# pfe-rs/lk-s-2022-estimacija-pokreta

Hardware: AMD Instinct MI355X
Metric: Mpix/s flow (1024x436, bcd_times=4) (higher is better)
Workload: dtype f64; 1 GPU; single 1024x436 Sintel-shape pair per step per GPU, forward only, bcd_times=4 (BASELINE.json configs[1]); cells 64x27, 150 labels/px; pairs_in_flight_per_gpu=7, mode=batch

## Files before the change

lk-s-2022-estimacija-pokreta_amd/csrc/knn_mfma.hip:

```cpp
#include "dflow_common.h"
#include "knn_pca.h"
#include "row_stage.h"

typedef _Float16 half8 __attribute__((ext_vector_type(8)));
typedef float f32x16 __attribute__((ext_vector_type(16)));

#define KM_ALPHA 64.0f
#define KM_K 48
#define KM_KSTEPS (KM_K / 16)
#define KM_KD 40
#define KM_SLOT_N 40
#define KM_SLOT_QE 41
#define KM_SLOT_EN 42
#define KM_SLOT_H 43
#define KM_SLOT_S 45
#define KM_SLOT_ONE 46
#define KM_XSCALE 64.0
#define KM_SSCALE 4096.0
#define KM_NORM2_MAX 30000.0
#define KM_WAVES 8
#define KM_THREADS (64 * KM_WAVES)
#define KM_QPW 64
#define KM_QPB (KM_WAVES * KM_QPW)
#ifndef KM_CHUNK
#define KM_CHUNK 192
#endif
#define KM_PITCH 112
#define KM_SLOTS (KM_PITCH / 16)
#define KM_STAGE_INS ((KM_CHUNK * KM_SLOTS + 63) / 64)
#define KM_ABUF (KM_STAGE_INS * 1024)
#ifndef KM_NBUF
#define KM_NBUF 3
#endif
#define KM_MAXNW ((KM_STAGE_INS + KM_WAVES - 1) / KM_WAVES)
#define KM_SPC (2 * (KM_CHUNK / 32))
#define KM_EVROWS_MAX 96
#define KM_MAXPTS 65535
#define KM_LIST_WORDS(evrows) (2 * (evrows) * 64)
#define KM_ETA 7.62939453125e-6

struct KmGeom {
    Geom g;
    int LP, qwaves;
    int evrows;
    float tphi;
};

__device__ static inline size_t list_id(const KmGeom &a, int qcell, int qwave, int wslot)
{
    const int win = 2 * a.g.win + 1;
    return ((size_t)qcell * a.qwaves + qwave) * (win * win) + wslot;
}

__host__ __device__ static inline int km_pad(int npts) { return (npts + KM_CHUNK - 1) / KM_CHUNK * KM_CHUNK; }
__host__ __device__ static inline int km_ntiles(int npts) { return km_pad(npts) / 32; }
__host__ __device__ static inline size_t km_cell_base(const Geom &g, int ci, int cj)
{
    const int wl = g.x1(g.ncx - 1) - g.x0(g.ncx - 1), hl = g.y1(g.ncy - 1) - g.y0(g.ncy - 1);
    const size_t rowsum = (size_t)(g.ncx - 1) * km_pad(g.cw * g.ch) + km_pad(wl * g.ch);
    const int hj = cj == g.ncy - 1 ? hl : g.ch;
    return (size_t)cj * rowsum + (size_t)ci * km_pad(g.cw * hj);
}
__host__ __device__ static inline size_t km_total_rows(const Geom &g)
{
    const int wl = g.x1(g.ncx - 1) - g.x0(g.ncx - 1), hl = g.y1(g.ncy - 1) - g.y0(g.ncy - 1);
    return km_cell_base(g, 0, g.ncy - 1) + (size_t)(g.ncx - 1) * km_pad(g.cw * hl) + km_pad(wl * hl);
}

__device__ static inline void km_store_sentinel(_Float16 *row)
{
    half8 *o = reinterpret_cast<half8 *>(row);
    const half8 z = {(_Float16)0.0f, (_Float16)0.0f, (_Float16)0.0f, (_Float16)0.0f, (_Float16)0.0f, (_Float16)0.0f, (_Float16)0.0f, (_Float16)0.0f};
    half8 t8 = z;
    t8[KM_SLOT_H - 40] = (_Float16)60000.0f;
#pragma unroll
    for (int k = 0; k < KM_K / 8; k++) o[k] = k == KM_K / 8 - 1 ? t8 : z;
}

__device__ static inline _Float16 km_f16_up(double v) { return (_Float16)(float)(v * 1.001 + 1e-7); }

#define KM_Q_ZERO 1.0f
#define KM_Q_BAD 2.0f
struct KmCellTop { uint32_t idx[5]; float cost[5]; };

#define KM_RHO 2.65e-5
typedef float km_f2p __attribute__((ext_vector_type(2)));
template <typename T>
__global__ void __launch_bounds__(256) knn_prep_kernel(const T *__restrict__ d1, const T *__restrict__ d2, const float *__restrict__ vt,
                                                       _Float16 *__restrict__ h1, _Float16 *__restrict__ h2,
                                                       float2 *__restrict__ qs, float2 *__restrict__ z0, uint8_t *__restrict__ zflag,
                                                       int *__restrict__ cell_bad, Geom g, int qblocks, int cblocks)
{
    const int which = (int)blockIdx.x >= qblocks ? 1 : 0;
    const T *__restrict__ d = which ? d2 : d1;
    _Float16 *__restrict__ h = which ? h2 : h1;
    const int cell = which ? ((int)blockIdx.x - qblocks) / cblocks : 0;
    int pix;
    size_t orow;
    if (which == 0) {
        pix = blockIdx.x * blockDim.x + threadIdx.x;
        if (pix >= g.H * g.W) return;
        orow = (size_t)pix;
    } else {
        const int ci = cell % g.ncx, cj = cell / g.ncx;
        const int cx0 = g.x0(ci), cy0 = g.y0(cj), ccw = g.x1(ci) - cx0, cnpts = ccw * (g.y1(cj) - cy0);
        const int pos = (((int)blockIdx.x - qblocks) % cblocks) * blockDim.x + threadIdx.x;
        if (pos >= km_pad(cnpts)) return;
        orow = km_cell_base(g, ci, cj) + pos;
        const int idx = (pos & 31) * km_ntiles(cnpts) + (pos >> 5);
        if (idx >= cnpts) {
            km_store_sentinel(h + orow * KM_K);
            z0[orow] = make_float2(INFINITY, 0.0f);
            zflag[orow] = 0;
            return;
        }
        pix = (cy0 + idx / ccw) * g.W + cx0 + idx % ccw;
    }
    float x[DFLOW_DESC];
    desc_load_row(x, d, (size_t)pix);
    if (which == 1) {
        const float4 zero[DFLOW_DESC / 4] = {};
        const PairDist zd = pair_dist(x, zero);
        z0[orow] = make_float2(zd.l2, zd.l1());
    }
    double sxall = 0.0;
    bool bad = false;
#pragma unroll
    for (int k = 0; k < DFLOW_DESC; k++) {
        const float sc = KM_ALPHA * x[k];
        bad |= (__float_as_uint(sc) & 0x7FFFFFFFu) >= 0x7F800000u;
        x[k] = sc;
        sxall = fma((double)sc, (double)sc, sxall);
    }
    bad |= !(sxall < KM_NORM2_MAX);
    const bool zero = sxall == 0.0;
    double ss = 0.0, sx = 0.0, se = 0.0;
    auto component = [&](int j) -> _Float16 {
        const km_f2p *__restrict__ vj = reinterpret_cast<const km_f2p *>(vt + (size_t)j * DFLOW_DESC);
        km_f2p acc = {0.0f, 0.0f};
#pragma unroll
        for (int i = 0; i < DFLOW_DESC / 2; i++) acc = __builtin_elementwise_fma(vj[i], (km_f2p){x[2 * i], x[2 * i + 1]}, acc);
        const float y = acc.x + acc.y;
        const _Float16 hv = (_Float16)y;
        const double f = (double)(float)hv, yd = (double)y, er = f - yd;
        ss = fma(f, f, ss); sx = fma(yd, yd, sx); se = fma(er, er, se);
        return hv;
    };
    half8 *o = reinterpret_cast<half8 *>(h + orow * KM_K);
    static_assert(KM_KD % 8 == 0 && KM_KD + 8 == KM_K, "the last 16-byte piece of a row holds the eight bound slots");
#pragma unroll 1
    for (int jo = 0; jo < KM_KD / 8; jo++) {
        half8 r;
#pragma unroll
        for (int j = 0; j < 8; j++) r[j] = component(8 * jo + j);
        o[jo] = r;
    }
    half8 last;
    const double rx = sqrt(sxall), ry = sqrt(sx);
    const double en = sqrt(se) + KM_RHO * rx;
    const double ypl = fmax(0.0, ry - KM_RHO * rx), ypu = ry + KM_RHO * rx;
    const double nd = sqrt(fmax(0.0, sxall * (1.0 + 1.1 * PCA_DELTA_MAX) - ypl * ypl));
    if (which == 0) {
        last[KM_SLOT_N - 40] = -km_f16_up(nd);
        last[KM_SLOT_QE - 40] = -km_f16_up(sqrt(ss) * (1.0 / KM_XSCALE));
        last[KM_SLOT_EN - 40] = -km_f16_up(en * KM_XSCALE);
        last[KM_SLOT_H - 40] = (_Float16)-1.0f; last[KM_SLOT_H + 1 - 40] = (_Float16)-1.0f;
        last[KM_SLOT_S - 40] = (_Float16)(float)(-1.0 / KM_SSCALE);
        last[KM_SLOT_ONE - 40] = (_Float16)0.0f; last[KM_SLOT_ONE + 1 - 40] = (_Float16)0.0f;
        qs[pix] = make_float2(bad ? KM_Q_BAD : zero ? KM_Q_ZERO : 0.0f, (float)(0.5 * sxall * (1.0 + 1.5 * PCA_DELTA_MAX) * 1.0000002));
    } else {
        const double hh = 0.5 * sxall;
        const _Float16 p1 = (_Float16)(float)hh;
        const _Float16 p2 = (_Float16)(float)(hh - (double)(float)p1);
        const double hres = fabs(hh - (double)(float)p1 - (double)(float)p2);
        const double scs = (KM_ETA * 1.001 * hh + 3e-6 * hh + hres) * 1.0004;
        last[KM_SLOT_N - 40] = km_f16_up(nd);
        last[KM_SLOT_QE - 40] = km_f16_up((en + KM_ETA * sqrt(ss)) * KM_XSCALE);
        last[KM_SLOT_EN - 40] = km_f16_up(ypu * (1.0 / KM_XSCALE));
        last[KM_SLOT_H - 40] = p1; last[KM_SLOT_H + 1 - 40] = p2;
        last[KM_SLOT_S - 40] = km_f16_up(scs * KM_SSCALE);
        last[KM_SLOT_ONE - 40] = (_Float16)1.0f; last[KM_SLOT_ONE + 1 - 40] = (_Float16)1.0f;
        zflag[orow] = zero ? 1 : 0;
        if (bad) cell_bad[cell] = 1;
    }
    o[KM_K / 8 - 1] = last;
}

__global__ void __launch_bounds__(256) knn_cell_post_kernel(_Float16 *__restrict__ h2, const float2 *__restrict__ z0,
                                                            const uint8_t *__restrict__ zflag, KmCellTop *__restrict__ ztop, Geom g)
{
    __shared__ int wsum[4];
    __shared__ unsigned long long wmin[4];
    const int ci = blockIdx.x % g.ncx, cj = blockIdx.x / g.ncx;
    const int cnpts = (g.x1(ci) - g.x0(ci)) * (g.y1(cj) - g.y0(cj));
    const int npad = km_pad(cnpts), ntiles = km_ntiles(cnpts);
    const size_t base = km_cell_base(g, ci, cj);
    const int tid = threadIdx.x, lane = tid & 63, wave = tid >> 6;
    int running = 0;
    for (int c0 = 0; c0 < cnpts; c0 += 256) {
        const int idx = c0 + tid;
        const int pos = (idx % ntiles) * 32 + idx / ntiles;
        const bool z = idx < cnpts && zflag[base + pos] != 0;
        const unsigned long long bal = __ballot(z);
        if (lane == 0) wsum[wave] = __popcll(bal);
        __syncthreads();
        int before = running + __popcll(bal & ((1ull << lane) - 1ull));
        int total = 0;
#pragma unroll
        for (int w = 0; w < 4; w++) { before += w < wave ? wsum[w] : 0; total += wsum[w]; }
        if (z && before >= 5) km_store_sentinel(h2 + (base + pos) * KM_K);
        running += total;
        __syncthreads();
    }
    unsigned long long k5[5];
#pragma unroll
    for (int i = 0; i < 5; i++) k5[i] = ~0ull;
    for (int pos = tid; pos < npad; pos += 256) {
        const int idx = (pos & 31) * ntiles + (pos >> 5);
        const float dd = z0[base + pos].x;
        if (idx < cnpts && dd < INFINITY) {
            unsigned long long x = ((unsigned long long)__float_as_uint(dd) << 32) | (unsigned)idx;
#pragma unroll
            for (int i = 0; i < 5; i++) { const bool lt = x < k5[i]; const unsigned long long lo = lt ? x : k5[i]; x = lt ? k5[i] : x; k5[i] = lo; }
        }
    }
    unsigned long long last = 0ull;
    bool first = true;
    for (int r = 0; r < 5; r++) {
        unsigned long long m = ~0ull;
#pragma unroll
        for (int i = 4; i >= 0; i--) if (first || k5[i] > last) m = k5[i];
        for (int off = 32; off > 0; off >>= 1) { const unsigned long long o = __shfl_xor(m, off); m = o < m ? o : m; }
        if (lane == 0) wmin[wave] = m;
        __syncthreads();
        m = wmin[0];
#pragma unroll
        for (int w = 1; w < 4; w++) m = wmin[w] < m ? wmin[w] : m;
        if (tid == 0) {
            const uint32_t idx = m == ~0ull ? 0u : (uint32_t)(m & 0xFFFFFFFFu);
            ztop[blockIdx.x].idx[r] = idx;
            ztop[blockIdx.x].cost[r] = z0[base + (idx % ntiles) * 32 + idx / ntiles].y;
        }
        last = m; first = false;
        __syncthreads();
    }
}

struct KmScreen {
    const _Float16 *h1, *h2;
    const float2 *qs;
    const int *cell_bad;
    uint32_t *ev;
    uint8_t *ev_cnt;
};

__device__ static inline void top5_insert_desc(float (&a)[5], float m)
{
#pragma unroll
    for (int i = 4; i >= 1; i--) a[i] = __builtin_amdgcn_fmed3f(a[i - 1], a[i], m);
    a[0] = fmaxf(a[0], m);
}

__device__ static inline float max16(const f32x16 &v)
{
    float m0 = fmaxf(fmaxf(v[0], v[1]), v[2]), m1 = fmaxf(fmaxf(v[3], v[4]), v[5]);
    float m2 = fmaxf(fmaxf(v[6], v[7]), v[8]), m3 = fmaxf(fmaxf(v[9], v[10]), v[11]);
    float m4 = fmaxf(fmaxf(v[12], v[13]), v[14]);
    return fmaxf(fmaxf(fmaxf(m0, m1), fmaxf(m2, m3)), fmaxf(m4, v[15]));
}

__global__ void __launch_bounds__(KM_THREADS, 4) knn_screen_kernel(KmGeom a, KmScreen p)
{
    extern __shared__ __attribute__((aligned(16))) char smem[];
    char *abuf = smem;

    const Geom g = a.g;
    const int tid = threadIdx.x, lane = tid & 63, wave = tid >> 6;
    const int col = lane & 31, half = lane >> 5;
    const int win = 2 * g.win + 1;
    const int wgs_per_cell = (win * win * a.qwaves + KM_WAVES - 1) / KM_WAVES;
    const int ccell = blockIdx.x / wgs_per_cell, w8 = blockIdx.x % wgs_per_cell;
    const int ci = ccell % g.ncx, cj = ccell / g.ncx;
    int flat = w8 * KM_WAVES + __builtin_amdgcn_readfirstlane(wave);
    int total = 0, qci = -1, qcj = -1, qwave = 0, fqci = -1, fqcj = -1;
    for (int qslot = 0; qslot < win * win; qslot++) {
        const int sci = ci - g.win + qslot / win, scj = cj - g.win + qslot % win;
        if (sci < 0 || sci >= g.ncx || scj < 0 || scj >= g.ncy) continue;
        const int nw = ((g.x1(sci) - g.x0(sci)) * (g.y1(scj) - g.y0(scj)) + KM_QPW - 1) / KM_QPW;
        if (fqci < 0) { fqci = sci; fqcj = scj; }
        if (qci < 0 && flat >= total && flat < total + nw) { qci = sci; qcj = scj; qwave = flat - total; }
        total += nw;
    }
    if (w8 * KM_WAVES >= total) return;
    const bool wave_active = qci >= 0;
    if (!wave_active) { qci = fqci; qcj = fqcj; qwave = 0; }
    const int qcell = qcj * g.ncx + qci;
    const int qx0 = g.x0(qci), qy0 = g.y0(qcj), qcw = g.x1(qci) - qx0, qnpts = qcw * (g.y1(qcj) - qy0);
    const int wslot = g.window(qci, qcj).slot(ci, cj);
    const int cx0 = g.x0(ci), cy0 = g.y0(cj), ccw = g.x1(ci) - cx0, cnpts = ccw * (g.y1(cj) - cy0);
    (void)cx0; (void)cy0;

    half8 bfrag[2][KM_KSTEPS];
    float hq[2];
    bool qzero[2], qbad = false;
#pragma unroll
    for (int gq = 0; gq < 2; gq++) {
        int qi = qwave * KM_QPW + gq * 32 + col;
        if (qi >= qnpts) qi = qnpts - 1;
        const int qpix = (qy0 + qi / qcw) * g.W + qx0 + qi % qcw;
        const half8 *src = reinterpret_cast<const half8 *>(p.h1 + (size_t)qpix * KM_K);
#pragma unroll
        for (int s = 0; s < KM_KSTEPS; s++) bfrag[gq][s] = src[2 * s + half];
        const float2 qq = p.qs[qpix];
        hq[gq] = qq.y;
        qzero[gq] = qq.x == KM_Q_ZERO;
        qbad |= qq.x == KM_Q_BAD;
    }
    const bool list_bad = __ballot(qbad) != 0ull || p.cell_bad[ccell] != 0;

    const int nchunks = (cnpts + KM_CHUNK - 1) / KM_CHUNK;
    const size_t cbase = km_cell_base(g, ci, cj);
    const int wave_u = __builtin_amdgcn_readfirstlane(wave);
    uint32_t soff[KM_MAXNW];
#pragma unroll
    for (int i = 0; i < KM_MAXNW; i++) {
        const int slot = (wave_u + i * KM_WAVES) * 64 + lane;
        int part = slot % KM_SLOTS;
        if (part >= KM_K / 8) part = 0;
        soff[i] = (uint32_t)((slot / KM_SLOTS) * (KM_K * 2) + part * 16);
    }
    const rs_gptr h2cell = (rs_gptr)(p.h2 + cbase * KM_K);
    const int n_w = (KM_STAGE_INS - wave_u + KM_WAVES - 1) / KM_WAVES;
    auto stage = [&](int chunk, int buf) {
        char *base = abuf + (size_t)buf * KM_ABUF + wave_u * 1024;
        const rs_gptr src = h2cell + (size_t)min(chunk, nchunks - 1) * (KM_CHUNK * KM_K * 2);
#pragma unroll
        for (int i = 0; i < KM_MAXNW; i++)
            if (i < KM_MAXNW - 1 || n_w == KM_MAXNW)
                __builtin_amdgcn_global_load_lds((const __attribute__((address_space(1))) void *)(src + soff[i]),
                                                 (__attribute__((address_space(3))) void *)(base + i * KM_WAVES * 1024), 16, 0, 0);
    };

    float a5[2][5];
    int cnt[2] = {0, 0};
    const int evrows = a.evrows;
    const uint32_t evoff[2] = {(uint32_t)lane * 4u, (uint32_t)lane * 4u + (uint32_t)evrows * 256u};
    const size_t lid = list_id(a, qcell, qwave, wslot);
    const __amdgpu_buffer_rsrc_t evrsrc = __builtin_amdgcn_make_buffer_rsrc((void *)(p.ev + lid * KM_LIST_WORDS(a.evrows)), 0, KM_LIST_WORDS(a.evrows) * 4, 0x00020000);

#pragma unroll
    for (int gq = 0; gq < 2; gq++)
#pragma unroll
        for (int i = 0; i < 5; i++) a5[gq][i] = -INFINITY;

    auto wait_ring = [&](int pass) {
        if (pass == 0) {
            if (n_w == KM_MAXNW) asm volatile("s_waitcnt vmcnt(%0)" ::"n"((KM_NBUF - 2) * KM_MAXNW) : "memory");
            else asm volatile("s_waitcnt vmcnt(%0)" ::"n"((KM_NBUF - 2) * (KM_MAXNW - 1)) : "memory");
        } else {
            if (n_w == KM_MAXNW) asm volatile("s_waitcnt vmcnt(%0)" ::"n"((KM_NBUF - 2) * KM_MAXNW + 2 * KM_SPC) : "memory");
            else asm volatile("s_waitcnt vmcnt(%0)" ::"n"((KM_NBUF - 2) * (KM_MAXNW - 1) + 2 * KM_SPC) : "memory");
        }
        __builtin_amdgcn_s_barrier();
    };
    auto dummy_stores = [&]() {
#pragma unroll
        for (int i = 0; i < KM_SPC; i++) __builtin_amdgcn_raw_buffer_store_b32(0u, evrsrc, (int)0xFFFFFF00u, 0, 0);
    };
    auto epi1 = [&](const f32x16 &acc, int gq) { top5_insert_desc(a5[gq], max16(acc)); };
    auto epi2 = [&](const f32x16 &acc, int gq, int tileidx) {
        uint32_t neg = 0u;
#pragma unroll
        for (int r = 15; r >= 0; r--) neg = __builtin_amdgcn_alignbit(neg, __float_as_uint(acc[r]), 31);
        const bool has = neg != 0xFFFFu;
        const uint32_t off = has ? evoff[gq] + ((uint32_t)min(cnt[gq], evrows - 1) << 8) : 0xFFFFFF00u;
        __builtin_amdgcn_raw_buffer_store_b32(neg ^ (((uint32_t)tileidx << 16) | 0xFFFFu), evrsrc, (int)off, 0, 0);
        cnt[gq] += has ? 1 : 0;
    };
    const f32x16 minus_inf = {-INFINITY, -INFINITY, -INFINITY, -INFINITY, -INFINITY, -INFINITY, -INFINITY, -INFINITY,
                              -INFINITY, -INFINITY, -INFINITY, -INFINITY, -INFINITY, -INFINITY, -INFINITY, -INFINITY};
    f32x16 pend;
    int pend_tile = 0;
    auto one_tile = [&](auto passc, const int tileidx, const half8 (&af)[KM_KSTEPS], half8 (&afn)[KM_KSTEPS], const char *arow_next) __attribute__((always_inline)) {
        constexpr int PASS = decltype(passc)::value;
        if (arow_next) {
#pragma unroll
            for (int s = 0; s < KM_KSTEPS; s++) afn[s] = *reinterpret_cast<const half8 *>(arow_next + s * 32);
        }
        __builtin_amdgcn_sched_barrier(0);
        f32x16 acc0 = {0.f, 0.f, 0.f, 0.f, 0.f, 0.f, 0.f, 0.f, 0.f, 0.f, 0.f, 0.f, 0.f, 0.f, 0.f, 0.f};
#pragma unroll
        for (int s = 0; s < KM_KSTEPS; s++) acc0 = __builtin_amdgcn_mfma_f32_32x32x16_f16(af[s], bfrag[0][s], acc0, 0, 0, 0);
        if (PASS == 0) epi1(pend, 1); else epi2(pend, 1, pend_tile);
#pragma unroll
        for (int s = 0; s < KM_KSTEPS; s++) {
            __builtin_amdgcn_sched_group_barrier(0x008, 1, 0);
            __builtin_amdgcn_sched_group_barrier(0x002, PASS == 0 ? 5 : 8, 0);
        }
        __builtin_amdgcn_sched_barrier(0);
        f32x16 acc1 = {0.f, 0.f, 0.f, 0.f, 0.f, 0.f, 0.f, 0.f, 0.f, 0.f, 0.f, 0.f, 0.f, 0.f, 0.f, 0.f};
#pragma unroll
        for (int s = 0; s < KM_KSTEPS; s++) acc1 = __builtin_amdgcn_mfma_f32_32x32x16_f16(af[s], bfrag[1][s], acc1, 0, 0, 0);
        if (PASS == 0) epi1(acc0, 0); else epi2(acc0, 0, tileidx);
#pragma unroll
        for (int s = 0; s < KM_KSTEPS; s++) {
            __builtin_amdgcn_sched_group_barrier(0x008, 1, 1);
            __builtin_amdgcn_sched_group_barrier(0x002, PASS == 0 ? 5 : 8, 1);
        }
        __builtin_amdgcn_sched_barrier(0);
        pend = acc1; pend_tile = tileidx;
    };
    auto tiles = [&](auto passc, const int chunk, const char *ab) __attribute__((always_inline)) {
        static_assert((KM_CHUNK / 32) % 2 == 1 || KM_CHUNK / 32 >= 2, "tiles per chunk");
        half8 afa[KM_KSTEPS], afb[KM_KSTEPS];
        const char *arow = ab + col * KM_PITCH + half * 16;
#pragma unroll
        for (int s = 0; s < KM_KSTEPS; s++) afa[s] = *reinterpret_cast<const half8 *>(arow + s * 32);
        const int tile0 = chunk * (KM_CHUNK / 32);
#pragma unroll 1
        for (int tile = 0; tile + 1 < KM_CHUNK / 32; tile += 2) {
            one_tile(passc, tile0 + tile, afa, afb, arow + (tile + 1) * 32 * KM_PITCH);
            one_tile(passc, tile0 + tile + 1, afb, afa, tile + 2 < KM_CHUNK / 32 ? arow + (tile + 2) * 32 * KM_PITCH : nullptr);
        }
        if ((KM_CHUNK / 32) % 2 == 1) one_tile(passc, tile0 + KM_CHUNK / 32 - 1, afa, afb, nullptr);
    };
    for (int pass = 0; pass < 2; pass++) {
#pragma unroll
        for (int c = 0; c < KM_NBUF - 1; c++) stage(c, c);
        if (n_w == KM_MAXNW) asm volatile("s_waitcnt vmcnt(%0)" ::"n"((KM_NBUF - 2) * KM_MAXNW) : "memory");
        else asm volatile("s_waitcnt vmcnt(%0)" ::"n"((KM_NBUF - 2) * (KM_MAXNW - 1)) : "memory");
        __builtin_amdgcn_s_barrier();
        pend = minus_inf;
        pend_tile = 0;
        if (pass == 1) dummy_stores();
        for (int chunk = 0; chunk < nchunks; chunk++) {
            const int buf = chunk % KM_NBUF;
            stage(chunk + KM_NBUF - 1, (chunk + KM_NBUF - 1) % KM_NBUF);
            const char *ab = abuf + (size_t)buf * KM_ABUF;
            if (wave_active) { if (pass == 0) tiles(IntC<0>(), chunk, ab); else tiles(IntC<1>(), chunk, ab); }
            else if (pass == 1) dummy_stores();
            wait_ring(pass);
        }
        if (wave_active) { if (pass == 0) epi1(pend, 1); else epi2(pend, 1, pend_tile); }
        asm volatile("s_waitcnt vmcnt(0)" ::: "memory");
        __builtin_amdgcn_s_barrier();
        if (pass == 0) {
#pragma unroll
            for (int gq = 0; gq < 2; gq++) {
                float o[5];
#pragma unroll
                for (int i = 0; i < 5; i++) o[i] = __shfl_xor(a5[gq][i], 32);
#pragma unroll
                for (int i = 0; i < 5; i++) top5_insert_desc(a5[gq], o[i]);
                const float a5v = a5[gq][4];
                const float x = a5v - 2.7e-5f * fmaxf(hq[gq] - a5v, 0.0f);
                float th = fmaxf(x - 1e-6f * (fabsf(a5v) + 2.7e-5f * hq[gq]), -55000.0f);
                if (qzero[gq]) th = 60000.0f;
                const float thp = th - 1e-5f * fabsf(th) - 6e-8f;
                if (half == 1) {
                    half8 b2 = bfrag[gq][KM_KSTEPS - 1];
                    b2[KM_SLOT_N - 40] = -b2[KM_SLOT_N - 40];
                    b2[KM_SLOT_QE - 40] = -b2[KM_SLOT_QE - 40];
                    b2[KM_SLOT_EN - 40] = -b2[KM_SLOT_EN - 40];
                    b2[KM_SLOT_S - 40] = -b2[KM_SLOT_S - 40];
                    const _Float16 p1 = (_Float16)thp;
                    const _Float16 p2 = (_Float16)(thp - (float)p1);
                    b2[KM_SLOT_ONE - 40] = -p1; b2[KM_SLOT_ONE + 1 - 40] = -p2;
                    bfrag[gq][KM_KSTEPS - 1] = b2;
                }
            }
        }
    }
    if (!wave_active) return;
#pragma unroll
    for (int gq = 0; gq < 2; gq++) p.ev_cnt[lid * 128 + gq * 64 + lane] = (uint8_t)(list_bad || cnt[gq] >= evrows ? 255 : cnt[gq]);
}

typedef unsigned int km_u4 __attribute__((ext_vector_type(4)));
struct RowDirectH {
    km_u4 r[9];
    __device__ __forceinline__ void init(char *, uint32_t *, int) {}
    __device__ __forceinline__ void issue(rs_gptr base, uint32_t off16, bool act)
    {
        if (act) {
            const __attribute__((address_space(1))) km_u4 *s = reinterpret_cast<const __attribute__((address_space(1))) km_u4 *>(base + ((unsigned long long)off16 << 4));
#pragma unroll
            for (int j = 0; j < 9; j++) r[j] = s[j];
        }
    }
    __device__ __forceinline__ void fetch(float4 (&cv)[17])
    {
        float f[72];
#pragma unroll
        for (int j = 0; j < 9; j++) {
            const dflow_h8 v = __builtin_bit_cast(dflow_h8, r[j]);
#pragma unroll
            for (int i = 0; i < 8; i++) f[8 * j + i] = (float)v[i];
        }
#pragma unroll
        for (int k = 0; k < 17; k++) cv[k] = make_float4(f[4 * k], f[4 * k + 1], f[4 * k + 2], f[4 * k + 3]);
    }
};
template <bool F16> struct RowsOf { typedef RowStage type; static constexpr uint32_t PIECES = 17u; };
template <> struct RowsOf<true> { typedef RowDirectH type; static constexpr uint32_t PIECES = 9u; };

struct KmResolve {
    const void *d1, *d2;
    const uint32_t *ev;
    const uint8_t *ev_cnt;
    const float2 *qs;
    const KmCellTop *ztop;
    uint32_t *proposals;
    float *lcosts;
    int *ovf_count;
    int4 *ovf_list;
    int ovf_cap;
    int *heavy_count;
    int4 *heavy_list;
    int heavy_cap;
};

__device__ static inline void key_insert(unsigned long long (&k)[5], float (&c)[5], unsigned long long x, float xc)
{
#pragma unroll
    for (int i = 0; i < 5; i++) {
        const bool lt = x < k[i];
        const unsigned long long lo = lt ? x : k[i], hi = lt ? k[i] : x;
        const float clo = lt ? xc : c[i], chi = lt ? c[i] : xc;
        k[i] = lo; c[i] = clo; x = hi; xc = chi;
    }
}
static constexpr unsigned long long KM_NO_KEY = 0x7F800000FFFFFFFFull;

__device__ static inline int km_event_cand(int h, int r, int tile, int ntiles) { return (4 * h + (r & 3) + 8 * (r >> 2)) * ntiles + tile; }

template <bool F16>
__device__ __forceinline__ void km_load_query(typename RowsOf<F16>::type &rows, const void *d1, size_t qpix, float (&q)[DFLOW_DESC])
{
    rows.issue((rs_gptr)d1, (uint32_t)qpix * RowsOf<F16>::PIECES, true);
    float4 qv[DFLOW_DESC / 4];
    rows.fetch(qv);
#pragma unroll
    for (int k = 0; k < DFLOW_DESC / 4; k++) { q[4 * k] = qv[k].x; q[4 * k + 1] = qv[k].y; q[4 * k + 2] = qv[k].z; q[4 * k + 3] = qv[k].w; }
}

template <class Rows, class Next>
__device__ __forceinline__ void km_eval(Rows &rows, Next &&next, const float (&q)[DFLOW_DESC], bool act, int idx,
                                        unsigned long long (&keys)[5], float (&costs)[5])
{
    float4 cv[DFLOW_DESC / 4];
    rows.fetch(cv);
    next();
    const float worst = __uint_as_float((unsigned)(keys[4] >> 32));
    const PairDist d = pair_dist(q, cv);
    if (act && !(d.l2 > worst)) key_insert(keys, costs, ((unsigned long long)__float_as_uint(d.l2) << 32) | (unsigned)idx, d.l1());
}

__device__ static inline void km_emit(const KmGeom &a, const KmResolve &p, size_t qpix, int qy, int qx, int cx0, int cy0, int ccw,
                                      int wslot, int j, unsigned long long key, float cost)
{
    const int idx = (int)(key & 0xFFFFFFFFu);
    const int ty = cy0 + idx / ccw, tx = cx0 + idx % ccw;
    p.proposals[qpix * a.LP + 5 * wslot + j] = pack_flow(ty - qy, tx - qx);
    p.lcosts[qpix * a.LP + 5 * wslot + j] = cost < a.tphi ? cost : a.tphi;
}

#ifndef KM_HEAVY_ENTRIES
#define KM_HEAVY_ENTRIES 32
#endif
#define KM_EVLIST2 30
typedef float km_f2 __attribute__((ext_vector_type(2)));
template <bool F16>
__global__ void __launch_bounds__(64, 2) knn_resolve_kernel(KmGeom a, KmResolve p)
{
    const Geom g = a.g;
    const int lane = threadIdx.x, gq = lane >> 5, col = lane & 31;
    const int win = 2 * g.win + 1;
    int b = blockIdx.x;
    const int qwave = b % a.qwaves; b /= a.qwaves;
    const int cir = b % win; const int qcell = b / win;
    const int qci = qcell % g.ncx, qcj = qcell / g.ncx;
    const int ci = qci - g.win + cir;
    if (ci < 0 || ci >= g.ncx) return;
    const int qx0 = g.x0(qci), qy0 = g.y0(qcj), qcw = g.x1(qci) - qx0, qnpts = qcw * (g.y1(qcj) - qy0);
    if (qwave * KM_QPW >= qnpts) return;
    const Geom::Window w = g.window(qci, qcj);
    const int cx0 = g.x0(ci), ccw = g.x1(ci) - cx0;

    __shared__ __attribute__((aligned(1024))) char stage[F16 ? 16 : ROW_STAGE_BYTES];
    __shared__ uint16_t evl[KM_EVLIST2][64];
    __shared__ __attribute__((aligned(16))) uint32_t s_cand[64];
    typename RowsOf<F16>::type rows;
    constexpr uint32_t PIECES = RowsOf<F16>::PIECES;
    rows.init(stage, s_cand, lane);
    float q[DFLOW_DESC];
    int qi = qwave * KM_QPW + lane;
    const bool qvalid = qi < qnpts;
    if (!qvalid) qi = qnpts - 1;
    const int qy = qy0 + qi / qcw, qx = qx0 + qi % qcw;
    const size_t qpix = (size_t)qy * g.W + qx;
    const bool qzero = p.qs[qpix].x == KM_Q_ZERO;
    km_load_query<F16>(rows, p.d1, qpix, q);
    const rs_gptr d2g = (rs_gptr)p.d2;

    int nA_n, nB_n; uint32_t entA_n[4], entB_n[4];
    auto prefetch = [&](int cj) {
        const size_t lid = list_id(a, qcell, qwave, w.slot(ci, cj));
        nA_n = p.ev_cnt[lid * 128 + gq * 64 + col]; nB_n = p.ev_cnt[lid * 128 + gq * 64 + col + 32];
        const uint32_t *ev = p.ev + lid * KM_LIST_WORDS(a.evrows) + (size_t)gq * a.evrows * 64 + col;
#pragma unroll
        for (int e = 0; e < 4; e++) { entA_n[e] = ev[e * 64]; entB_n[e] = ev[e * 64 + 32]; }
    };
    prefetch(w.jmin);
    for (int cj = w.jmin; cj <= w.jmax; cj++) {
        const int wslot = w.slot(ci, cj);
        const size_t lid = list_id(a, qcell, qwave, wslot);
        const int cy0 = g.y0(cj);
        const int ntiles = km_ntiles(ccw * (g.y1(cj) - cy0));
        int nA = nA_n, nB = nB_n;
        bool ovf = nA == 255 || nB == 255;
        const uint32_t *evA = p.ev + (size_t)lid * KM_LIST_WORDS(a.evrows) + (size_t)gq * a.evrows * 64 + col;
        uint32_t entA[4], entB[4];
#pragma unroll
        for (int e = 0; e < 4; e++) { entA[e] = e < nA && !ovf ? entA_n[e] : 0u; entB[e] = e < nB && !ovf ? entB_n[e] : 0u; }
        if (cj < w.jmax) prefetch(cj + 1);
        if (__ballot(ovf)) {
            if (lane == 0) {
                int pos = atomicAdd(p.ovf_count, 1);
                if (pos < p.ovf_cap) p.ovf_list[pos] = make_int4(qcell, qwave * KM_QPW, ci, cj);
            }
            continue;
        }
        bool heavy = false;
        if (nA + nB > KM_HEAVY_ENTRIES) {
            heavy = true;
            if (qvalid) {
                const int pos = atomicAdd(p.heavy_count, 1);
                if (pos < p.heavy_cap) p.heavy_list[pos] = make_int4(qcell, qi, ci, cj); else heavy = false;
            }
            if (heavy) {
                nA = 0; nB = 0;
#pragma unroll
                for (int e = 0; e < 4; e++) { entA[e] = 0u; entB[e] = 0u; }
            }
        }
        unsigned long long keys[5];
        float costs[5];
#pragma unroll
        for (int i = 0; i < 5; i++) { keys[i] = KM_NO_KEY; costs[i] = 0.0f; }
        int done = 0, total;
        do {
        int nev = 0, seen = 0;
        auto expand = [&](uint32_t entry, int h) {
            const int tile = (int)(entry >> 16);
            uint32_t mask = entry & 0xFFFFu;
            while (mask) {
                const int r = __ffs(mask) - 1;
                mask &= mask - 1;
                if (seen >= done && nev < KM_EVLIST2) { evl[nev][lane] = (uint16_t)km_event_cand(h, r, tile, ntiles); nev++; }
                seen++;
            }
        };
#pragma unroll
        for (int e = 0; e < 4; e++) expand(entA[e], 0);
        for (int e = 4; e < nA; e++) expand(evA[e * 64], 0);
#pragma unroll
        for (int e = 0; e < 4; e++) expand(entB[e], 1);
        for (int e = 4; e < nB; e++) expand(evA[e * 64 + 32], 1);
        total = seen;
        auto issue_cand = [&](int e) -> int {
            const bool act = e < nev;
            const int idx = act ? evl[e][lane] : 0;
            rows.issue(d2g, (uint32_t)((cy0 + idx / ccw) * g.W + cx0 + idx % ccw) * PIECES, act);
            return idx;
        };
        if (__ballot(nev > 0)) {
            int e = 0;
            int idx_next = issue_cand(0);
            while (true) {
                const bool act = e < nev;
                const int idx = idx_next;
                e++;
                const bool more = __ballot(e < nev) != 0;
                km_eval(rows, [&] { if (more) idx_next = issue_cand(e); }, q, act, idx, keys, costs);
                if (!more) break;
            }
        }
        done += nev;
        } while (__ballot(done < total));
        if (qzero) {
            const KmCellTop zt = p.ztop[cj * g.ncx + ci];
#pragma unroll
            for (int i = 0; i < 5; i++) { keys[i] = zt.idx[i]; costs[i] = zt.cost[i]; }
        }
        if (qvalid && !heavy) {
#pragma unroll
            for (int j = 0; j < 5; j++) km_emit(a, p, qpix, qy, qx, cx0, cy0, ccw, wslot, j, keys[j], costs[j]);
        }
    }
}

#define KM_HEAVY_CAND 1024
template <bool F16>
__global__ void __launch_bounds__(64, 2) knn_resolve_heavy_kernel(KmGeom a, KmResolve p)
{
    const Geom g = a.g;
    const int lane = threadIdx.x;
    __shared__ __attribute__((aligned(1024))) char stage[F16 ? 16 : ROW_STAGE_BYTES];
    __shared__ __attribute__((aligned(16))) uint32_t s_cand[64];
    __shared__ uint16_t cand[KM_HEAVY_CAND];
    typename RowsOf<F16>::type rows;
    constexpr uint32_t PIECES = RowsOf<F16>::PIECES;
    rows.init(stage, s_cand, lane);
    const int nitems = min(*p.heavy_count, p.heavy_cap);
    const rs_gptr d2g = (rs_gptr)p.d2;
    for (int item = blockIdx.x; item < nitems; item += gridDim.x) {
        const int4 it = p.heavy_list[item];
        const int qcell = it.x, qi = it.y, ci = it.z, cj = it.w;
        const int qci = qcell % g.ncx, qcj = qcell / g.ncx;
        const int qx0 = g.x0(qci), qy0 = g.y0(qcj), qcw = g.x1(qci) - qx0;
        const int qy = qy0 + qi / qcw, qx = qx0 + qi % qcw;
        const size_t qpix = (size_t)qy * g.W + qx;
        const int wslot = g.window(qci, qcj).slot(ci, cj);
        const int cx0 = g.x0(ci), cy0 = g.y0(cj), ccw = g.x1(ci) - cx0;
        const int ntiles = km_ntiles(ccw * (g.y1(cj) - cy0));
        const size_t lid = list_id(a, qcell, qi / KM_QPW, wslot);
        const int ql = qi % KM_QPW, gq = ql >> 5, col = ql & 31;
        const uint32_t *ev = p.ev + (size_t)lid * KM_LIST_WORDS(a.evrows) + (size_t)gq * a.evrows * 64 + col;
        const int nA = p.ev_cnt[lid * 128 + gq * 64 + col], nB = p.ev_cnt[lid * 128 + gq * 64 + col + 32];
        const int te = min(lane, a.evrows - 1);
        const uint32_t pre_a = ev[(size_t)te * 64], pre_b = ev[(size_t)te * 64 + 32];
        float q[DFLOW_DESC];
        km_load_query<F16>(rows, p.d1, qpix, q);
        unsigned long long keys[5];
        float costs[5];
#pragma unroll
        for (int i = 0; i < 5; i++) { keys[i] = KM_NO_KEY; costs[i] = 0.0f; }
        for (int e0 = 0; e0 < nA + nB; e0 += 64) {
            const int t = e0 + lane;
            uint32_t en = 0u; int h = 0;
            const uint32_t shb = (uint32_t)__shfl((int)pre_b, (t - nA) & 63);
            if (t < nA) en = t < 64 ? pre_a : ev[(size_t)t * 64];
            else if (t < nA + nB) { en = t - nA < 64 ? shb : ev[(size_t)(t - nA) * 64 + 32]; h = 1; }
            const int cntl = t < nA + nB ? __popc(en & 0xFFFFu) : 0;
            int incl = cntl;
#pragma unroll
            for (int off = 1; off < 64; off <<= 1) { const int v = __shfl_up(incl, off); if (lane >= off) incl += v; }
            const int nc = __shfl(incl, 63);
            {
                int o = incl - cntl;
                const int tile = (int)(en >> 16);
                uint32_t m = t < nA + nB ? (en & 0xFFFFu) : 0u;
                while (m) { const int r = __ffs(m) - 1; m &= m - 1; cand[o++] = (uint16_t)km_event_cand(h, r, tile, ntiles); }
            }
            asm volatile("s_waitcnt lgkmcnt(0)" ::: "memory");
            auto issue_cand = [&](int c0) -> int {
                const bool act = c0 + lane < nc;
                const int idx = act ? cand[c0 + lane] : 0;
                rows.issue(d2g, (uint32_t)((cy0 + idx / ccw) * g.W + cx0 + idx % ccw) * PIECES, act);
                return idx;
            };
            int idx_next = issue_cand(0);
            for (int c0 = 0; c0 < nc; c0 += 64) {
                const int idx = idx_next;
                km_eval(rows, [&] { if (c0 + 64 < nc) idx_next = issue_cand(c0 + 64); }, q, c0 + lane < nc, idx, keys, costs);
            }
        }
        unsigned long long rkey = KM_NO_KEY;
        float rcost = 0.0f;
        for (int r = 0; r < 5; r++) {
            unsigned long long m = keys[0];
#pragma unroll
            for (int off = 32; off > 0; off >>= 1) { const unsigned long long o = __shfl_xor(m, off); m = o < m ? o : m; }
            const unsigned long long own = __ballot(keys[0] == m && m != KM_NO_KEY);
            float c = 0.0f;
            if (own) {
                const int wl = __ffsll((long long)own) - 1;
                c = __shfl(costs[0], wl);
                if (lane == wl) {
#pragma unroll
                    for (int i = 0; i < 4; i++) { keys[i] = keys[i + 1]; costs[i] = costs[i + 1]; }
                    keys[4] = KM_NO_KEY; costs[4] = 0.0f;
                }
            }
            if (lane == r) { rkey = m; rcost = c; }
        }
        if (lane < 5) km_emit(a, p, qpix, qy, qx, cx0, cy0, ccw, wslot, lane, rkey, rcost);
    }
}

template <int CTRL> __device__ static inline void dpp_lexmin(float &mind, int &best)
{
    const float om = __builtin_bit_cast(float, __builtin_amdgcn_update_dpp(__builtin_bit_cast(int, mind), __builtin_bit_cast(int, mind), CTRL, 0xF, 0xF, false));
    const int ob = __builtin_amdgcn_update_dpp(best, best, CTRL, 0xF, 0xF, false);
    if (om < mind || (om == mind && ob < best)) { mind = om; best = ob; }
}
__global__ void __launch_bounds__(256) knn_finalize_kernel(Geom g, int LP, uint32_t *__restrict__ proposals, float *__restrict__ lcosts,
                                                           int32_t *__restrict__ nprop, int32_t *__restrict__ bestlabels)
{
    const int sub = threadIdx.x & 15;
    const int pix = (blockIdx.x * blockDim.x + threadIdx.x) >> 4;
    const bool ok = pix < g.H * g.W;
    const int px = ok ? pix : 0;
    const int cy = g.celly(px / g.W), cx = g.cellx(px % g.W);
    const int wy = min(g.ncy - 1, cy + g.win) - max(0, cy - g.win) + 1;
    const int wx = min(g.ncx - 1, cx + g.win) - max(0, cx - g.win) + 1;
    const int n = 5 * wy * wx;
    const float *lc = lcosts + (size_t)px * LP;
    float mind = 1000.0f; int best = 0x7fffffff;
    float cs[DFLOW_MAX_LABELS / 16];
#pragma unroll
    for (int j = 0; j < DFLOW_MAX_LABELS / 16; j++) cs[j] = sub + 16 * j < n ? lc[sub + 16 * j] : 1000.0f;
#pragma unroll
    for (int j = 0; j < DFLOW_MAX_LABELS / 16; j++) if (cs[j] < mind) { mind = cs[j]; best = sub + 16 * j; }
    dpp_lexmin<0x101>(mind, best); dpp_lexmin<0x102>(mind, best); dpp_lexmin<0x104>(mind, best); dpp_lexmin<0x108>(mind, best);
    if (ok) {
        if (sub == 0) { nprop[pix] = n; bestlabels[pix] = best == 0x7fffffff ? 0 : best; }
        for (int l = n + sub; l < LP; l += 16) { proposals[(size_t)pix * LP + l] = DFLOW_FILL_PROPOSAL; lcosts[(size_t)pix * LP + l] = DFLOW_FILL_COST; }
    }
}

static size_t num_lists(const dflow_params *p)
{
    Geom g = make_geom(p);
    size_t qwaves = (max_cell_points(g) + KM_QPW - 1) / KM_QPW, win = 2 * g.win + 1;
    return (size_t)g.ncx * g.ncy * qwaves * win * win;
}

#define KM_HEAVY_BLOCKS 2048
#define KM_HEAVY_CAP (1 << 20)
static int km_evrows(const dflow_params *p)
{
    const int tiles = km_ntiles(max_cell_points(make_geom(p)));
    return tiles + 1 < KM_EVROWS_MAX ? tiles + 1 : KM_EVROWS_MAX;
}

struct KmWs {
    _Float16 *h1, *h2;
    float2 *qs, *z0;
    uint8_t *zflag;
    int *ctr;
    int *cell_bad;
    size_t zero_bytes;
    float *vt;
    void *pca_ws;
    KmCellTop *ztop;
    int4 *ovf;
    int4 *heavy;
    uint32_t *ev;
    uint8_t *ev_cnt;
    size_t nl, bytes;
    int evrows;
};

static KmWs km_ws(const dflow_params *p, void *ws)
{
    const Geom g = make_geom(p);
    const size_t N = (size_t)g.H * g.W, rows2 = km_total_rows(g), ncells = (size_t)g.ncx * g.ncy;
    WsCarver c(ws);
    KmWs k;
    k.nl = num_lists(p);
    k.evrows = km_evrows(p);
    k.h1 = c.take<_Float16>(N * KM_K);
    k.h2 = c.take<_Float16>(rows2 * KM_K);
    k.qs = c.take<float2>(N);
    k.z0 = c.take<float2>(rows2);
    k.zflag = c.take<uint8_t>(rows2);
    k.zero_bytes = 256 + ncells * sizeof(int);
    k.ctr = c.take<int>(k.zero_bytes / sizeof(int));
    k.cell_bad = k.ctr + 256 / sizeof(int);
    k.vt = c.take<float>(DFLOW_DESC * DFLOW_DESC);
    k.pca_ws = c.take<char>(knn_pca_ws_bytes());
    k.ztop = c.take<KmCellTop>(ncells);
    k.ovf = c.take<int4>(k.nl);
    k.heavy = c.take<int4>(KM_HEAVY_CAP);
    k.ev = c.take<uint32_t>(k.nl * KM_LIST_WORDS(k.evrows));
    k.ev_cnt = c.take<uint8_t>(k.nl * 128);
    k.bytes = c.bytes;
    return k;
}

size_t knn_mfma_ws_bytes(const dflow_params *p) { return km_ws(p, nullptr).bytes; }

static KmGeom km_geom(const dflow_params *p, const KmWs &k)
{
    KmGeom a;
    a.g = make_geom(p); a.LP = p->label_pitch; a.tphi = p->tphi;
    a.qwaves = (max_cell_points(a.g) + KM_QPW - 1) / KM_QPW;
    a.evrows = k.evrows;
    return a;
}

bool knn_mfma_supported(const dflow_params *p)
{
    Geom g = make_geom(p);
    return max_cell_points(g) <= KM_MAXPTS && p->window >= 0 && p->window <= 2;
}

#define KM_MARK(i) do { if (tev) DFLOW_HIP(hipEventRecord(tev[i], s)); } while (0)
int launch_knn_mfma(const dflow_params *p, const void *d1, const void *d2, uint32_t *proposals, float *lcosts,
                    int32_t *nprop, int32_t *bestlabels, void *ws, hipStream_t s, hipEvent_t *tev)
{
    Geom g = make_geom(p);
    const size_t N = (size_t)g.H * g.W;
    const KmWs k = km_ws(p, ws);
    DFLOW_HIP(hipMemsetAsync(k.ctr, 0, k.zero_bytes, s));
    int nb = (int)((N + 255) / 256);
    KM_MARK(0);
    int rc = launch_knn_pca(p, d2, k.vt, k.ctr + 1, k.pca_ws, s);
    if (rc) return rc;
    KM_MARK(1);
    const int cblocks = (km_pad(max_cell_points(g)) + 255) / 256;
    with_descr_type(p, [&](auto d) {
        using T = typename decltype(d)::T;
        hipLaunchKernelGGL(knn_prep_kernel<T>, dim3(nb + cblocks * g.ncx * g.ncy), dim3(256), 0, s, (const T *)d1, (const T *)d2, (const float *)k.vt,
                           k.h1, k.h2, k.qs, k.z0, k.zflag, k.cell_bad, g, nb, cblocks);
    });
    hipLaunchKernelGGL(knn_cell_post_kernel, dim3(g.ncx * g.ncy), dim3(256), 0, s, k.h2, (const float2 *)k.z0, (const uint8_t *)k.zflag, k.ztop, g);
    rc = dflow_check_launch("knn_cell_post_kernel");
    if (rc) return rc;

    KM_MARK(2);
    const KmGeom a = km_geom(p, k);
    int win = 2 * g.win + 1;
    int wgs_per_cell = (win * win * a.qwaves + KM_WAVES - 1) / KM_WAVES;
    KmScreen sc;
    sc.h1 = k.h1; sc.h2 = k.h2; sc.qs = k.qs; sc.cell_bad = k.cell_bad; sc.ev = k.ev; sc.ev_cnt = k.ev_cnt;
    size_t shmem = (size_t)KM_NBUF * KM_ABUF;
    hipLaunchKernelGGL(knn_screen_kernel, dim3(g.ncx * g.ncy * wgs_per_cell), dim3(KM_THREADS), shmem, s, a, sc);
    rc = dflow_check_launch("knn_screen_kernel");
    if (rc) return rc;
    KM_MARK(3);
    KmResolve rs;
    rs.d1 = d1; rs.d2 = d2; rs.ev = k.ev; rs.ev_cnt = k.ev_cnt; rs.qs = k.qs; rs.ztop = k.ztop; rs.proposals = proposals; rs.lcosts = lcosts;
    rs.ovf_count = k.ctr; rs.ovf_list = k.ovf; rs.ovf_cap = (int)k.nl;
    rs.heavy_count = k.ctr + 2; rs.heavy_list = k.heavy; rs.heavy_cap = KM_HEAVY_CAP;
    const dim3 rgrid((unsigned)(g.ncx * g.ncy * win * a.qwaves));
    with_descr_type(p, [&](auto d) { hipLaunchKernelGGL(knn_resolve_kernel<decltype(d)::F16>, rgrid, dim3(64), 0, s, a, rs); });
    rc = dflow_check_launch("knn_resolve_kernel");
    if (rc) return rc;
    with_descr_type(p, [&](auto d) { hipLaunchKernelGGL(knn_resolve_heavy_kernel<decltype(d)::F16>, dim3(KM_HEAVY_BLOCKS), dim3(64), 0, s, a, rs); });
    rc = dflow_check_launch("knn_resolve_heavy_kernel");
    if (rc) return rc;
    KM_MARK(4);
    rc = launch_knn_fix(p, d1, d2, proposals, lcosts, k.ctr, k.ovf, (int)k.nl, k.ctr + 1, s);
    if (rc) return rc;
    KM_MARK(5);
    hipLaunchKernelGGL(knn_finalize_kernel, dim3((unsigned)((N * 16 + 255) / 256)), dim3(256), 0, s, g, a.LP, proposals, lcosts, nprop, bestlabels);
    KM_MARK(6);
    return dflow_check_launch("knn_finalize_kernel");
}
#undef KM_MARK

__global__ void __launch_bounds__(128) knn_stats_lists_kernel(KmGeom a, const uint32_t *__restrict__ ev, const uint8_t *__restrict__ ev_cnt,
                                                              unsigned long long *__restrict__ out)
{
    const Geom g = a.g;
    const int evrows = a.evrows, win = 2 * g.win + 1;
    const size_t lid = blockIdx.x;
    {
        const int wslot = (int)(lid % (size_t)(win * win)), qwave = (int)(lid / (win * win) % a.qwaves), qcell = (int)(lid / (win * win) / a.qwaves);
        const int qci = qcell % g.ncx, qcj = qcell / g.ncx;
        const Geom::Window w = g.window(qci, qcj);
        const int qnpts = (g.x1(qci) - g.x0(qci)) * (g.y1(qcj) - g.y0(qcj));
        if (qwave * KM_QPW >= qnpts || wslot >= (w.imax - w.imin + 1) * (w.jmax - w.jmin + 1)) return;
    }
    const int gq = threadIdx.x >> 6, lane = threadIdx.x & 63;
    const int cnt = ev_cnt[lid * 128 + threadIdx.x];
    unsigned long long entries = 0, events = 0;
    if (cnt != 255) {
        entries = (unsigned long long)cnt;
        const uint32_t *e = ev + lid * KM_LIST_WORDS(evrows) + (size_t)gq * evrows * 64 + lane;
        for (int i = 0; i < cnt; i++) events += (unsigned long long)__popc(e[i * 64] & 0xFFFFu);
    }
    unsigned long long mx = entries;
    for (int off = 32; off > 0; off >>= 1) { entries += __shfl_xor(entries, off); events += __shfl_xor(events, off); const unsigned long long o = __shfl_xor(mx, off); mx = o > mx ? o : mx; }
    if (lane == 0) { atomicAdd(out + 0, entries); atomicAdd(out + 1, events); atomicMax(out + 2, mx); }
}

__global__ void __launch_bounds__(256) knn_stats_rows_kernel(const float2 *__restrict__ qs, int npix, const uint8_t *__restrict__ zflag,
                                                             const _Float16 *__restrict__ h2, size_t rows2, unsigned long long *__restrict__ out)
{
    const size_t i = (size_t)blockIdx.x * blockDim.x + threadIdx.x;
    const bool zq = i < (size_t)npix && qs[i].x == KM_Q_ZERO, bq = i < (size_t)npix && qs[i].x == KM_Q_BAD;
    const bool zc = i < rows2 && zflag[i] != 0;
    const bool removed = zc && h2[i * KM_K + KM_SLOT_H] == (_Float16)60000.0f;
    const unsigned long long b0 = __ballot(zq), b1 = __ballot(bq), b2 = __ballot(zc), b3 = __ballot(removed);
    if ((threadIdx.x & 63) == 0) {
        if (b0) atomicAdd(out + 3, (unsigned long long)__popcll(b0));
        if (b1) atomicAdd(out + 4, (unsigned long long)__popcll(b1));
        if (b2) atomicAdd(out + 5, (unsigned long long)__popcll(b2));
        if (b3) atomicAdd(out + 6, (unsigned long long)__popcll(b3));
    }
}

int knn_mfma_stats(const dflow_params *p, void *ws, hipStream_t s, int64_t *h_out)
{
    const KmWs k = km_ws(p, ws);
    const Geom g = make_geom(p);
    const size_t N = (size_t)g.H * g.W, rows2 = km_total_rows(g);
    unsigned long long *dev = (unsigned long long *)(k.ctr + 16);
    DFLOW_HIP(hipMemsetAsync(dev, 0, 8 * sizeof(unsigned long long), s));
    const KmGeom a = km_geom(p, k);
    hipLaunchKernelGGL(knn_stats_lists_kernel, dim3((unsigned)k.nl), dim3(128), 0, s, a, (const uint32_t *)k.ev, (const uint8_t *)k.ev_cnt, dev);
    const size_t m = N > rows2 ? N : rows2;
    hipLaunchKernelGGL(knn_stats_rows_kernel, dim3((unsigned)((m + 255) / 256)), dim3(256), 0, s, (const float2 *)k.qs, (int)N, (const uint8_t *)k.zflag,
                       (const _Float16 *)k.h2, rows2, dev);
    int rc = dflow_check_launch("knn_stats kernels");
    if (rc) return rc;
    unsigned long long c[8];
    int ctr[4];
    DFLOW_HIP(hipMemcpyAsync(c, dev, sizeof(c), hipMemcpyDeviceToHost, s));
    DFLOW_HIP(hipMemcpyAsync(ctr, k.ctr, sizeof(ctr), hipMemcpyDeviceToHost, s));
    DFLOW_HIP(hipStreamSynchronize(s));
    long long pairs = 0;
    for (int qcj = 0; qcj < g.ncy; qcj++)
        for (int qci = 0; qci < g.ncx; qci++) {
            const long long qn = (long long)(g.x1(qci) - g.x0(qci)) * (g.y1(qcj) - g.y0(qcj));
            const Geom::Window w = g.window(qci, qcj);
            pairs += qn * (w.imax - w.imin + 1) * (w.jmax - w.jmin + 1);
        }
    h_out[0] = ctr[0]; h_out[1] = ctr[1]; h_out[2] = (int64_t)k.nl; h_out[3] = (int64_t)c[0]; h_out[4] = (int64_t)c[1]; h_out[5] = (int64_t)c[2];
    h_out[6] = (int64_t)c[3]; h_out[7] = (int64_t)c[4]; h_out[8] = (int64_t)c[5]; h_out[9] = (int64_t)c[6]; h_out[10] = pairs; h_out[11] = k.evrows;
    h_out[12] = ctr[2] < KM_HEAVY_CAP ? ctr[2] : KM_HEAVY_CAP;
    h_out[13] = ctr[2] > KM_HEAVY_CAP ? ctr[2] - KM_HEAVY_CAP : 0;
    return DFLOW_OK;
}

double knn_mfma_issued(const dflow_params *p)
{
    Geom g = make_geom(p);
    double n = 0.0;
    for (int qcj = 0; qcj < g.ncy; qcj++)
        for (int qci = 0; qci < g.ncx; qci++) {
            const int qnpts = (g.x1(qci) - g.x0(qci)) * (g.y1(qcj) - g.y0(qcj));
            const int qgroups = 2 * ((qnpts + KM_QPW - 1) / KM_QPW);
            for (int ci = qci - g.win; ci <= qci + g.win; ci++)
                for (int cj = qcj - g.win; cj <= qcj + g.win; cj++) {
                    if (ci < 0 || ci >= g.ncx || cj < 0 || cj >= g.ncy) continue;
                    const int cnpts = (g.x1(ci) - g.x0(ci)) * (g.y1(cj) - g.y0(cj));
                    n += (double)qgroups * km_ntiles(cnpts) * 2.0 * KM_KSTEPS;
                }
        }
    return n;
}
```

Before: 40.90 Mpix/s.

## Restructure kNN MFMA chunk ring to stage one chunk ahead with optional wave lag

Reworks the LDS staging ring in the MFMA kNN kernel. It now prefetches only the next chunk instead of NBUF-1 ahead, waits on vmcnt(0) or just the pending store count, and walks tiles by a global tile index that wraps around the contiguous ring. It adds an optional lag for the upper half of the waves so that their reads skew against the lower half, and it sizes the dummy stores to match the real epilogue stores so the vmcnt bookkeeping stays consistent. The aim is simpler, tighter synchronization and staggered wave progress. The risk is less prefetch depth and more exposed global latency.

```diff
diff --git a/lk-s-2022-estimacija-pokreta_amd/csrc/knn_mfma.hip b/lk-s-2022-estimacija-pokreta_amd/csrc/knn_mfma.hip
--- a/lk-s-2022-estimacija-pokreta_amd/csrc/knn_mfma.hip
+++ b/lk-s-2022-estimacija-pokreta_amd/csrc/knn_mfma.hip
@@ -32,8 +32,19 @@
 #ifndef KM_NBUF
 #define KM_NBUF 3
 #endif
+#ifndef KM_LAG
+#define KM_LAG 0
+#endif
+#define KM_TPC (KM_CHUNK / 32)
+#define KM_TILE_BYTES (32 * KM_PITCH)
+#define KM_RING_TILES (KM_NBUF * KM_TPC)
 #define KM_MAXNW ((KM_STAGE_INS + KM_WAVES - 1) / KM_WAVES)
-#define KM_SPC (2 * (KM_CHUNK / 32))
+#define KM_SPC (2 * KM_TPC)
+static_assert(KM_ABUF == KM_TPC * KM_TILE_BYTES, "the ring is contiguous in tiles: tile T of a cell sits at (T % KM_RING_TILES) * KM_TILE_BYTES");
+static_assert(KM_TPC % 2 == 0 && KM_LAG % 2 == 0, "tiles go in pairs (the tile loop is unrolled by two over its two fragment sets)");
+static_assert(KM_LAG >= 0 && KM_LAG < KM_TPC, "a late wave reads chunks c - 1 and c in interval c, nothing older");
+static_assert(KM_NBUF >= 3, "chunk c + 1 is staged while chunks c - 1 (late waves) and c are read");
+static_assert(KM_SPC <= 63, "vmcnt is a 6-bit counter");
 #define KM_EVROWS_MAX 96
 #define KM_MAXPTS 65535
 #define KM_LIST_WORDS(evrows) (2 * (evrows) * 64)
@@ -333,7 +344,7 @@
     const int n_w = (KM_STAGE_INS - wave_u + KM_WAVES - 1) / KM_WAVES;
     auto stage = [&](int chunk, int buf) {
         char *base = abuf + (size_t)buf * KM_ABUF + wave_u * 1024;
-        const rs_gptr src = h2cell + (size_t)min(chunk, nchunks - 1) * (KM_CHUNK * KM_K * 2);
+        const rs_gptr src = h2cell + (size_t)chunk * (KM_CHUNK * KM_K * 2);
 #pragma unroll
         for (int i = 0; i < KM_MAXNW; i++)
             if (i < KM_MAXNW - 1 || n_w == KM_MAXNW)
@@ -354,18 +365,12 @@
         for (int i = 0; i < 5; i++) a5[gq][i] = -INFINITY;
 
     auto wait_ring = [&](int pass) {
-        if (pass == 0) {
-            if (n_w == KM_MAXNW) asm volatile("s_waitcnt vmcnt(%0)" ::"n"((KM_NBUF - 2) * KM_MAXNW) : "memory");
-            else asm volatile("s_waitcnt vmcnt(%0)" ::"n"((KM_NBUF - 2) * (KM_MAXNW - 1)) : "memory");
-        } else {
-            if (n_w == KM_MAXNW) asm volatile("s_waitcnt vmcnt(%0)" ::"n"((KM_NBUF - 2) * KM_MAXNW + 2 * KM_SPC) : "memory");
-            else asm volatile("s_waitcnt vmcnt(%0)" ::"n"((KM_NBUF - 2) * (KM_MAXNW - 1) + 2 * KM_SPC) : "memory");
-        }
+        if (pass == 0) asm volatile("s_waitcnt vmcnt(0)" ::: "memory");
+        else asm volatile("s_waitcnt vmcnt(%0)" ::"n"(KM_SPC) : "memory");
         __builtin_amdgcn_s_barrier();
     };
-    auto dummy_stores = [&]() {
-#pragma unroll
-        for (int i = 0; i < KM_SPC; i++) __builtin_amdgcn_raw_buffer_store_b32(0u, evrsrc, (int)0xFFFFFF00u, 0, 0);
+    auto dummy_stores = [&](int first) {
+        for (int i = first; i < KM_SPC; i++) __builtin_amdgcn_raw_buffer_store_b32(0u, evrsrc, (int)(0xFFFFFF00u - ((uint32_t)i << 8)), 0, 0);
     };
     auto epi1 = [&](const f32x16 &acc, int gq) { top5_insert_desc(a5[gq], max16(acc)); };
     auto epi2 = [&](const f32x16 &acc, int gq, int tileidx) {
@@ -381,9 +386,9 @@
                               -INFINITY, -INFINITY, -INFINITY, -INFINITY, -INFINITY, -INFINITY, -INFINITY, -INFINITY};
     f32x16 pend;
     int pend_tile = 0;
-    auto one_tile = [&](auto passc, const int tileidx, const half8 (&af)[KM_KSTEPS], half8 (&afn)[KM_KSTEPS], const char *arow_next) __attribute__((always_inline)) {
+    auto one_tile = [&](auto passc, const int tileidx, const half8 (&af)[KM_KSTEPS], half8 (&afn)[KM_KSTEPS], const bool fetch_next, const char *arow_next) __attribute__((always_inline)) {
         constexpr int PASS = decltype(passc)::value;
-        if (arow_next) {
+        if (fetch_next) {
 #pragma unroll
             for (int s = 0; s < KM_KSTEPS; s++) afn[s] = *reinterpret_cast<const half8 *>(arow_next + s * 32);
         }
@@ -410,36 +415,38 @@
         __builtin_amdgcn_sched_barrier(0);
         pend = acc1; pend_tile = tileidx;
     };
-    auto tiles = [&](auto passc, const int chunk, const char *ab) __attribute__((always_inline)) {
-        static_assert((KM_CHUNK / 32) % 2 == 1 || KM_CHUNK / 32 >= 2, "tiles per chunk");
+    auto tiles = [&](auto passc, const int tb, const int te) __attribute__((always_inline)) {
+        if (tb >= te) return;
         half8 afa[KM_KSTEPS], afb[KM_KSTEPS];
-        const char *arow = ab + col * KM_PITCH + half * 16;
-#pragma unroll
-        for (int s = 0; s < KM_KSTEPS; s++) afa[s] = *reinterpret_cast<const half8 *>(arow + s * 32);
-        const int tile0 = chunk * (KM_CHUNK / 32);
+        const char *arow = abuf + col * KM_PITCH + half * 16;
+        auto next = [](int o) { return o + KM_TILE_BYTES == KM_RING_TILES * KM_TILE_BYTES ? 0 : o + KM_TILE_BYTES; };
+        int off = (tb % KM_RING_TILES) * KM_TILE_BYTES;
+#pragma unroll
+        for (int s = 0; s < KM_KSTEPS; s++) afa[s] = *reinterpret_cast<const half8 *>(arow + off + s * 32);
 #pragma unroll 1
-        for (int tile = 0; tile + 1 < KM_CHUNK / 32; tile += 2) {
-            one_tile(passc, tile0 + tile, afa, afb, arow + (tile + 1) * 32 * KM_PITCH);
-            one_tile(passc, tile0 + tile + 1, afb, afa, tile + 2 < KM_CHUNK / 32 ? arow + (tile + 2) * 32 * KM_PITCH : nullptr);
-        }
-        if ((KM_CHUNK / 32) % 2 == 1) one_tile(passc, tile0 + KM_CHUNK / 32 - 1, afa, afb, nullptr);
+        for (int tile = tb; tile < te; tile += 2) {
+            const int off1 = next(off);
+            off = next(off1);
+            one_tile(passc, tile, afa, afb, true, arow + off1);
+            one_tile(passc, tile + 1, afb, afa, tile + 2 < te, arow + off);
+        }
     };
+    const int lag = wave_u >= KM_WAVES / 2 ? KM_LAG : 0;
+    const int ntl = nchunks * KM_TPC;
     for (int pass = 0; pass < 2; pass++) {
-#pragma unroll
-        for (int c = 0; c < KM_NBUF - 1; c++) stage(c, c);
-        if (n_w == KM_MAXNW) asm volatile("s_waitcnt vmcnt(%0)" ::"n"((KM_NBUF - 2) * KM_MAXNW) : "memory");
-        else asm volatile("s_waitcnt vmcnt(%0)" ::"n"((KM_NBUF - 2) * (KM_MAXNW - 1)) : "memory");
+        stage(0, 0);
+        asm volatile("s_waitcnt vmcnt(0)" ::: "memory");
         __builtin_amdgcn_s_barrier();
         pend = minus_inf;
         pend_tile = 0;
-        if (pass == 1) dummy_stores();
-        for (int chunk = 0; chunk < nchunks; chunk++) {
-            const int buf = chunk % KM_NBUF;
-            stage(chunk + KM_NBUF - 1, (chunk + KM_NBUF - 1) % KM_NBUF);
-            const char *ab = abuf + (size_t)buf * KM_ABUF;
-            if (wave_active) { if (pass == 0) tiles(IntC<0>(), chunk, ab); else tiles(IntC<1>(), chunk, ab); }
-            else if (pass == 1) dummy_stores();
-            wait_ring(pass);
+        for (int c = 0; c <= nchunks; c++) {
+            if (c + 1 < nchunks) stage(c + 1, (c + 1) % KM_NBUF);
+            const int tb = max(c * KM_TPC - lag, 0), te = min((c + 1) * KM_TPC - lag, ntl);
+            if (wave_active) { if (pass == 0) tiles(IntC<0>(), tb, te); else tiles(IntC<1>(), tb, te); }
+            if (c + 1 < nchunks) {
+                if (pass == 1) dummy_stores(wave_active ? 2 * (te - tb) : 0);
+                wait_ring(pass);
+            }
         }
         if (wave_active) { if (pass == 0) epi1(pend, 1); else epi2(pend, 1, pend_tile); }
         asm volatile("s_waitcnt vmcnt(0)" ::: "memory");
```

Result: no change. 41.15 Mpix/s (median of 5 runs) (+0.6%).
